# k-flouris/cmf

Hardware: AMD Instinct MI355X
Metric: log-density evals/sec (JtJ-cholesky path), MNIST D=784 d=64 bs=512 (higher is better)
Workload: dtype f32 (3x3 tangent convs as bf16x3 split MFMA, fp32 accumulate); 1 GPU; C3: MNIST-shaped (1,28,28) uint8-range + U[0,1) noise, non-square flow d=64, cholesky J^T J log-det + g_ij off-diagonal L1 + reconstruction, eval/no_grad; per_gpu_batch=512, global_batch=512, D=784, latent_dimension=64, parallelism=dp1

## Files before the change

### cmf_amd/csrc/conv_head.hip

```cpp
#include <stdint.h>

#include "common.h"

namespace {

constexpr int HID = 64, KJ = HID * 9, NT = 192, ACC = 16;
constexpr int SLICE = HID * 16;

__device__ __forceinline__ int out_pixel(int po, int W, int live) {
  if (!live) return po;
  const int wh = W >> 1, row = po / wh, k = po - row * wh;
  return row * W + 2 * k + ((row + live - 1) & 1);
}

template <int CP>
__global__ __launch_bounds__(NT, CP == 8 ? 2 : 3) void conv_head_kernel(cmf_conv_tangent_args a, int n_out, int tiles_per_sample, int ntiles) {
  constexpr int P = ACC / CP;
  __shared__ __attribute__((aligned(16))) float Es[P * KJ * CP];
  __shared__ __attribute__((aligned(16))) float Gs[HID * ACC];
  __shared__ unsigned long long um[P * 9];
  __shared__ unsigned long long alv[P];
  __shared__ int pixs[P];

  const int per = (ntiles + 7) >> 3;
  const int item = (int)(blockIdx.x & 7) * per + (int)(blockIdx.x >> 3);
  if (item >= ntiles) return;
  const int b = item / tiles_per_sample, p0 = (item - b * tiles_per_sample) * P;
  const int cnt = n_out - p0 < P ? n_out - p0 : P;
  const int tid = threadIdx.x, lane = tid & 63, wv = tid >> 6;
  const int H = a.H, W = a.W, cout = a.head_cout;

  if (tid < P * 9) {
    const int p = tid / 9, tap = tid - p * 9;
    unsigned long long m = 0;
    if (p < cnt) {
      const int pix = out_pixel(p0 + p, W, a.live);
      const int r = pix / W + tap / 3 - 1, c = pix % W + tap % 3 - 1;
      if (r >= 0 && r < H && c >= 0 && c < W)
        m = *reinterpret_cast<const unsigned long long*>(reinterpret_cast<const unsigned char*>(a.f) + (long long)b * a.f_np +
                                                         (long long)(r * W + c) * (HID / 8));
    }
    um[tid] = m;
  }
  for (int p = wv; p < P; p += NT / 64) {
    const int pix = p < cnt ? out_pixel(p0 + p, W, a.live) : 0;
    bool on = false;
    if (p < cnt) on = a.head_a[(long long)b * a.head_a_np + (long long)lane * a.head_a_c + (long long)pix * a.head_a_px] > 0.f;
    const unsigned long long bal = __ballot(on);
    if (lane == 0) {
      alv[p] = bal;
      pixs[p] = pix;
    }
#pragma unroll
    for (int o = 0; o < CP; ++o) Gs[(lane * P + p) * CP + o] = (on && o < cout) ? a.head_w[o * HID + lane] : 0.f;
  }
  __syncthreads();

  {
    static_assert(3 * NT == KJ, "three (ci, tap) pairs per thread");
    float acc[3][ACC];
#pragma unroll
    for (int r = 0; r < 3; ++r)
#pragma unroll
      for (int i = 0; i < ACC; ++i) acc[r][i] = 0.f;
#pragma unroll 2
    for (int c = 0; c < HID; ++c) {
      float w[3];
#pragma unroll
      for (int r = 0; r < 3; ++r) w[r] = a.w[c * KJ + tid + r * NT];
#pragma unroll
      for (int i = 0; i < ACC / 4; ++i) {
        const f32x4 g = *reinterpret_cast<const f32x4*>(&Gs[c * ACC + 4 * i]);
#pragma unroll
        for (int r = 0; r < 3; ++r)
#pragma unroll
          for (int k = 0; k < 4; ++k) acc[r][4 * i + k] = fmaf(g[k], w[r], acc[r][4 * i + k]);
      }
    }
#pragma unroll
    for (int r = 0; r < 3; ++r)
#pragma unroll
      for (int p = 0; p < P; ++p)
#pragma unroll
        for (int o = 0; o < CP; ++o) Es[(p * KJ + tid + r * NT) * CP + o] = acc[r][p * CP + o];
  }
  __syncthreads();

  const int nsl = a.nc >> 4, cl = lane >> 2;
  const f32x4 zero = {0.f, 0.f, 0.f, 0.f};
  for (int unit = wv; unit < nsl * P; unit += NT / 64) {
    const int sl = unit / P, p = unit - sl * P;
    if (p >= cnt) continue;
    const int pix = pixs[p];
    const float* hb = a.r + (long long)b * a.r_np + (long long)pix * a.r_px + sl * SLICE + lane * 4;
    const float* ub = a.x + (long long)b * a.x_np + sl * SLICE + lane * 4;
    f32x4 acc[CP];
#pragma unroll
    for (int o = 0; o < CP; ++o) acc[o] = zero;

    auto load4 = [&](f32x4* v, const float* src, unsigned long long m) {
#pragma unroll
      for (int ch = 0; ch < 4; ++ch) {
        v[ch] = zero;
        if ((m >> (ch * 16 + cl)) & 1) v[ch] = *reinterpret_cast<const f32x4*>(src + ch * 256);
      }
    };
    auto load_row = [&](f32x4* v, int ty) {
#pragma unroll
      for (int tx = 0; tx < 3; ++tx)
        load4(v + 4 * tx, ub + (long long)(pix + (ty - 1) * W + (tx - 1)) * a.x_px, um[p * 9 + ty * 3 + tx]);
    };
    auto fma4 = [&](const f32x4* v, const float* coef, int stride) {
#pragma unroll
      for (int ch = 0; ch < 4; ++ch) {
        const float* e4 = static_cast<const float*>(__builtin_assume_aligned(coef + ch * stride, CP < 4 ? 8 : 16));
#pragma unroll
        for (int o = 0; o < CP; ++o) {
          const float e = e4[o];
#pragma unroll
          for (int k = 0; k < 4; ++k) acc[o][k] = fmaf(e, v[ch][k], acc[o][k]);
        }
      }
    };
    auto fma_row = [&](const f32x4* v, int ty) {
#pragma unroll
      for (int tx = 0; tx < 3; ++tx) fma4(v + 4 * tx, &Es[(p * KJ + cl * 9 + ty * 3 + tx) * CP], 16 * 9 * CP);
    };
    {
      f32x4 vh[4], v[12];
      load4(vh, hb, alv[p]);
      load_row(v, 0);
      fma4(vh, &Gs[(cl * P + p) * CP], 16 * P * CP);
      fma_row(v, 0);
    }
#pragma unroll 1
    for (int ty = 1; ty < 3; ++ty) {
      f32x4 v[12];
      load_row(v, ty);
      fma_row(v, ty);
    }

    constexpr int N = 4 * CP;
    float val[N];
#pragma unroll
    for (int o = 0; o < CP; ++o)
#pragma unroll
      for (int k = 0; k < 4; ++k) val[4 * o + k] = acc[o][k];
#pragma unroll
    for (int s = 0; s < 4; ++s) {
      const int off = 32 >> s, n = N >> s;
      if (n >= 2) {
        const bool hi = lane & off;
#pragma unroll
        for (int i = 0; i < n / 2; ++i) {
          const float mine = hi ? val[n / 2 + i] : val[i], send = hi ? val[i] : val[n / 2 + i];
          val[i] = mine + __shfl_xor(send, off, 64);
        }
      } else {
        val[0] += __shfl_xor(val[0], off, 64);
      }
    }
    float* yb = a.head_y + (long long)b * a.head_y_np + (long long)(p0 + p) * a.head_y_px + sl * 16 + (lane & 3) * 4;
    constexpr int KEEP = N >= 16 ? N / 16 : 1;
#pragma unroll
    for (int i = 0; i < KEEP; ++i) {
      const int idx = ((cl * N) >> 4) + i, o = idx >> 2;
      if (o < cout && (N >= 16 || !(lane & 4))) yb[(long long)o * a.head_y_co + (idx & 3)] = val[i];
    }
  }
}

template <int CP>
int launch(const cmf_conv_tangent_args& a, hipStream_t s) {
  constexpr int P = ACC / CP;
  const int n_out = a.live ? a.H * a.W / 2 : a.H * a.W;
  const long long tiles = (n_out + P - 1) / P, ntiles = tiles * a.np;
  if (ntiles > 0x7ffffff0LL) return CMF_ERANGE;
  const int grid = 8 * (int)((ntiles + 7) / 8);
  hipLaunchKernelGGL(conv_head_kernel<CP>, dim3(grid), dim3(NT), 0, s, a, n_out, (int)tiles, (int)ntiles);
  CMF_LAUNCH_CHECK();
  return 0;
}

}

int cmf_conv_head(const cmf_conv_tangent_args& a, hipStream_t s) {
  if (!a.x || !a.w || !a.f || !a.r || !a.head_w || !a.head_a || !a.head_y) return CMF_EINVAL;
  if (a.fmode != CMF_F_RELU_BITS || a.taps != 9 || a.cin != HID || a.cout != HID) return CMF_EINVAL;
  if (a.head_cout < 1 || a.head_cout > 8 || a.np <= 0 || a.H <= 0 || a.W <= 0 || a.nc <= 0 || a.nc % 16) return CMF_EINVAL;
  if (a.bias || a.fo || a.ymask || a.mask_out || a.live < 0 || a.live > 2 || (a.live && a.W % 2)) return CMF_EINVAL;
  if (!((a.W % 14 == 0 && a.H % 2 == 0) || (a.W % 8 == 0 && a.H % 4 == 0))) return CMF_EINVAL;
  const long long HW = (long long)a.H * a.W;
  if (HW > (1 << 24)) return CMF_ERANGE;
  if (a.x_ci != 16 || a.x_sl != SLICE || a.r_co != 16 || a.r_sl != SLICE) return CMF_EINVAL;
  if ((a.x_np | a.x_px | a.r_np | a.r_px | a.head_y_np | a.head_y_co | a.head_y_px) % 4) return CMF_EINVAL;
  if (a.x_px < (long long)HID * a.nc || a.r_px < (long long)HID * a.nc || a.head_y_px < a.nc) return CMF_EINVAL;
  if ((uintptr_t)a.x % 16 || (uintptr_t)a.r % 16 || (uintptr_t)a.head_y % 16 || (uintptr_t)a.w % 4 || (uintptr_t)a.head_w % 4) return CMF_EINVAL;
  if ((uintptr_t)a.f % 8 || a.f_np % 8 || a.f_np < HW * (HID / 8)) return CMF_EINVAL;
  const int cp = a.head_cout <= 2 ? 2 : a.head_cout <= 4 ? 4 : 8;
  return cp == 2 ? launch<2>(a, s) : cp == 4 ? launch<4>(a, s) : launch<8>(a, s);
}
```

Baseline: 1489 evals/s.

## Deduplicate conv-head tap loads and pipeline them with a buffer-load ring

The conv head kernel now builds a per-tile table of unique input pixels shared across the P output pixels' 3x3 neighbourhoods, so overlapping taps are loaded once and applied to every output that uses them. Loads go through raw buffer_load instructions with out-of-range offsets standing in for masked lanes, issued into a three-deep register ring so global loads overlap FMA work. A fourth wave is added that prefetches while the other three compute the E coefficients, and the E layout in LDS is padded (stride 11) to hold the head weights as a tenth tap. This adds considerable complexity, inline asm with hand-set waitcnts, and higher register pressure under the same launch bounds.

Result: no change. 1492 evals/s (median of 6 runs) (+0.2%).

```diff
diff --git a/cmf_amd/csrc/conv_head.hip b/cmf_amd/csrc/conv_head.hip
--- a/cmf_amd/csrc/conv_head.hip
+++ b/cmf_amd/csrc/conv_head.hip
@@ -1,11 +1,19 @@
 #include <stdint.h>
 
+#include <type_traits>
+
 #include "common.h"
 
 namespace {
 
-constexpr int HID = 64, KJ = HID * 9, NT = 192, ACC = 16;
+constexpr int HID = 64, KJ = HID * 9, NT = 256, NW = NT / 64, NTB = 192, ACC = 16;
 constexpr int SLICE = HID * 16;
+constexpr int ES = 11;
+constexpr int RING = 3;
+constexpr int NENT = 128;
+constexpr int X_DROP = 0x7ffffff0;
+
+typedef int i32x4 __attribute__((ext_vector_type(4)));
 
 __device__ __forceinline__ int out_pixel(int po, int W, int live) {
   if (!live) return po;
@@ -13,51 +21,194 @@
   return row * W + 2 * k + ((row + live - 1) & 1);
 }
 
+__device__ __forceinline__ i32x4 block_rsrc(const float* p) {
+  const unsigned long long u = reinterpret_cast<unsigned long long>(p);
+  i32x4 d;
+  d[0] = __builtin_amdgcn_readfirstlane((int)(unsigned)u);
+  d[1] = __builtin_amdgcn_readfirstlane((int)((unsigned)(u >> 32) & 0xffffu));
+  d[2] = SLICE * 4;
+  d[3] = 0x00020000;
+  return d;
+}
+
 template <int CP>
 __global__ __launch_bounds__(NT, CP == 8 ? 2 : 3) void conv_head_kernel(cmf_conv_tangent_args a, int n_out, int tiles_per_sample, int ntiles) {
   constexpr int P = ACC / CP;
-  __shared__ __attribute__((aligned(16))) float Es[P * KJ * CP];
+  __shared__ __attribute__((aligned(16))) float Es[P * HID * ES * CP];
   __shared__ __attribute__((aligned(16))) float Gs[HID * ACC];
-  __shared__ unsigned long long um[P * 9];
-  __shared__ unsigned long long alv[P];
-  __shared__ int pixs[P];
+  __shared__ __attribute__((aligned(16))) unsigned ent[NENT][4];
+  __shared__ int keys[P * 9], fst[P * 9], nent_s;
 
   const int per = (ntiles + 7) >> 3;
   const int item = (int)(blockIdx.x & 7) * per + (int)(blockIdx.x >> 3);
   if (item >= ntiles) return;
   const int b = item / tiles_per_sample, p0 = (item - b * tiles_per_sample) * P;
   const int cnt = n_out - p0 < P ? n_out - p0 : P;
-  const int tid = threadIdx.x, lane = tid & 63, wv = tid >> 6;
+  const int tid = threadIdx.x, lane = tid & 63, wv = __builtin_amdgcn_readfirstlane(tid >> 6);
   const int H = a.H, W = a.W, cout = a.head_cout;
 
+  constexpr int NOKEY = 0x7fffffff;
+  const bool narrow = W + 2 <= 64;
+  int key = NOKEY, kq = 0;
+  unsigned long long km = 0;
   if (tid < P * 9) {
     const int p = tid / 9, tap = tid - p * 9;
-    unsigned long long m = 0;
     if (p < cnt) {
       const int pix = out_pixel(p0 + p, W, a.live);
       const int r = pix / W + tap / 3 - 1, c = pix % W + tap % 3 - 1;
-      if (r >= 0 && r < H && c >= 0 && c < W)
-        m = *reinterpret_cast<const unsigned long long*>(reinterpret_cast<const unsigned char*>(a.f) + (long long)b * a.f_np +
-                                                         (long long)(r * W + c) * (HID / 8));
-    }
-    um[tid] = m;
-  }
-  for (int p = wv; p < P; p += NT / 64) {
+      key = (r + 1) * (W + 2) + c + 1;
+      if (r >= 0 && r < H && c >= 0 && c < W) {
+        kq = r * W + c;
+        km = *reinterpret_cast<const unsigned long long*>(reinterpret_cast<const unsigned char*>(a.f) + (long long)b * a.f_np +
+                                                          (long long)kq * (HID / 8));
+      }
+      if (narrow) {
+        const int wh = a.live ? W >> 1 : W, row0 = p0 / wh;
+        int row = row0, k = p0 - row0 * wh;
+        unsigned long long rows[4] = {0, 0, 0, 0};
+        unsigned code = ~0u;
+#pragma unroll
+        for (int i = 0; i < P; ++i) {
+          if (i < cnt) {
+            const int col = a.live ? 2 * k + ((row + a.live - 1) & 1) : k, d = row - row0;
+            const unsigned long long w3 = 7ull << col;
+#pragma unroll
+            for (int x = 0; x < 4; ++x)
+              if (x >= d && x <= d + 2) rows[x] |= w3;
+            const int dr = r - row, dc = c - col;
+            if (dr >= -1 && dr <= 1 && dc >= -1 && dc <= 1) code = (code & ~(0xfu << (4 * i))) | ((unsigned)((dr + 1) * 3 + dc + 1) << (4 * i));
+            if (++k == wh) {
+              k = 0;
+              ++row;
+            }
+          }
+        }
+        const int rr = r - row0 + 1;
+        int rank = 0, n = 0;
+#pragma unroll
+        for (int x = 0; x < 4; ++x) {
+          n += __popcll(rows[x]);
+          rank += x < rr ? __popcll(rows[x]) : x == rr ? __popcll(rows[x] & ((1ull << (c + 1)) - 1)) : 0;
+        }
+        const int j = cnt + rank;
+        ent[j][0] = (unsigned)kq;
+        ent[j][1] = (unsigned)km;
+        ent[j][2] = (unsigned)(km >> 32);
+        ent[j][3] = code;
+        if (tid == 0) nent_s = cnt + n;
+      }
+    }
+    keys[tid] = key;
+  }
+  if (!narrow && tid >= cnt && tid < NENT) ent[tid][3] = ~0u;
+  for (int p = wv; p < P; p += NW) {
     const int pix = p < cnt ? out_pixel(p0 + p, W, a.live) : 0;
     bool on = false;
     if (p < cnt) on = a.head_a[(long long)b * a.head_a_np + (long long)lane * a.head_a_c + (long long)pix * a.head_a_px] > 0.f;
     const unsigned long long bal = __ballot(on);
-    if (lane == 0) {
-      alv[p] = bal;
-      pixs[p] = pix;
-    }
-#pragma unroll
-    for (int o = 0; o < CP; ++o) Gs[(lane * P + p) * CP + o] = (on && o < cout) ? a.head_w[o * HID + lane] : 0.f;
+    if (lane == 0 && p < cnt) {
+      ent[p][0] = (unsigned)pix | 0x80000000u;
+      ent[p][1] = (unsigned)bal;
+      ent[p][2] = (unsigned)(bal >> 32);
+      ent[p][3] = ~(0xfu << (4 * p)) | (9u << (4 * p));
+    }
+#pragma unroll
+    for (int o = 0; o < CP; ++o) {
+      const float g = (on && o < cout) ? a.head_w[o * HID + lane] : 0.f;
+      Gs[(lane * P + p) * CP + o] = g;
+      Es[((p * HID + lane) * ES + 9) * CP + o] = g;
+    }
   }
   __syncthreads();
-
-  {
-    static_assert(3 * NT == KJ, "three (ci, tap) pairs per thread");
+  if (!narrow) {
+    if (tid < P * 9) {
+      int first = key != NOKEY;
+      for (int t = 0; t < P * 9; ++t) first &= !(t < tid && keys[t] == key);
+      fst[tid] = first;
+    }
+    __syncthreads();
+    if (tid < P * 9) {
+      int rank = 0, n = 0;
+      for (int t = 0; t < P * 9; ++t) {
+        rank += fst[t] & (keys[t] < key);
+        n += fst[t];
+      }
+      if (tid == 0) nent_s = cnt + n;
+      if (key != NOKEY) {
+        const int p = tid / 9, tap = tid - p * 9, j = cnt + rank;
+        if (fst[tid]) {
+          ent[j][0] = (unsigned)kq;
+          ent[j][1] = (unsigned)km;
+          ent[j][2] = (unsigned)(km >> 32);
+        }
+        atomicAnd(&ent[j][3], ~(0xfu << (4 * p)) | ((unsigned)tap << (4 * p)));
+      }
+    }
+    __syncthreads();
+  }
+
+  const int nsl = a.nc >> 4;
+  const int nent = __builtin_amdgcn_readfirstlane(nent_s);
+  const int lsub = nsl >= 3 ? 0 : nsl == 2 ? 1 : (P < NW ? 1 : 2);
+  const int psub = P >> lsub, nunits = nsl << lsub;
+  const i32x4 e0 = *reinterpret_cast<const i32x4*>(ent[lane]), e1 = *reinterpret_cast<const i32x4*>(ent[lane + 64]);
+  auto field = [&](int j, int k) {
+    if constexpr (P * 10 <= 64) {
+      return (unsigned)__builtin_amdgcn_readlane(e0[k], j);
+    } else {
+      const int lo = __builtin_amdgcn_readlane(e0[k], j & 63), hi = __builtin_amdgcn_readlane(e1[k], j & 63);
+      return (unsigned)(j < 64 ? lo : hi);
+    }
+  };
+  auto others = [&](int u) { return ~(unsigned)(((1ull << (4 * psub)) - 1) << (4 * psub * (u & ((1 << lsub) - 1)))); };
+  const f32x4 zero = {0.f, 0.f, 0.f, 0.f};
+  int lcl = lane >> 2;
+  asm volatile("" : "+v"(lcl));
+  const int loff = lane * 16;
+  const unsigned bit0 = 1u << lcl, bit1 = 0x10000u << lcl;
+  const long long xpx = a.x_px, rpx = a.r_px;
+  f32x4 ring[RING][4];
+  int iu = wv, ij = 0;
+  const float *ixb = a.x, *irb = a.r;
+  unsigned iot = 0;
+  auto issue_unit = [&]() {
+    const int u = iu < nunits ? iu : 0;
+    ixb = a.x + (long long)b * a.x_np + (u >> lsub) * SLICE;
+    irb = a.r + (long long)b * a.r_np + (u >> lsub) * SLICE;
+    iot = others(u);
+  };
+  issue_unit();
+  auto issue = [&](f32x4 (&v)[4]) {
+    const bool valid = iu < nunits;
+    const int j = valid ? ij : 0;
+    const unsigned e = field(j, 0);
+    const bool need = valid && (lsub == 0 || (field(j, 3) | iot) != ~0u);
+    const unsigned mlo = need ? field(j, 1) : 0u, mhi = need ? field(j, 2) : 0u;
+    const long long pixel = (long long)(e & 0x7fffffffu);
+    const float* src = (e >> 31) ? irb + pixel * rpx : ixb + pixel * xpx;
+    const i32x4 rs = block_rsrc(src);
+    const int o0 = mlo & bit0 ? loff : X_DROP, o1 = mlo & bit1 ? loff : X_DROP;
+    const int o2 = mhi & bit0 ? loff : X_DROP, o3 = mhi & bit1 ? loff : X_DROP;
+    asm volatile(
+        "s_nop 4\n\t"
+        "buffer_load_dwordx4 %0, %4, %8, 0 offen\n\t"
+        "buffer_load_dwordx4 %1, %5, %8, 0 offen offset:1024\n\t"
+        "buffer_load_dwordx4 %2, %6, %8, 0 offen offset:2048\n\t"
+        "buffer_load_dwordx4 %3, %7, %8, 0 offen offset:3072"
+        : "=&v"(v[0]), "=&v"(v[1]), "=&v"(v[2]), "=&v"(v[3])
+        : "v"(o0), "v"(o1), "v"(o2), "v"(o3), "s"(rs)
+        : "memory");
+    if (valid && ++ij == nent) {
+      ij = 0;
+      iu += NW;
+      issue_unit();
+    }
+  };
+#pragma unroll
+  for (int s = 0; s < RING; ++s) issue(ring[s]);
+
+  if (tid < NTB) {
+    static_assert(3 * NTB == KJ, "three (ci, tap) pairs per thread");
     float acc[3][ACC];
 #pragma unroll
     for (int r = 0; r < 3; ++r)
@@ -67,7 +218,7 @@
     for (int c = 0; c < HID; ++c) {
       float w[3];
 #pragma unroll
-      for (int r = 0; r < 3; ++r) w[r] = a.w[c * KJ + tid + r * NT];
+      for (int r = 0; r < 3; ++r) w[r] = a.w[c * KJ + tid + r * NTB];
 #pragma unroll
       for (int i = 0; i < ACC / 4; ++i) {
         const f32x4 g = *reinterpret_cast<const f32x4*>(&Gs[c * ACC + 4 * i]);
@@ -78,96 +229,106 @@
       }
     }
 #pragma unroll
-    for (int r = 0; r < 3; ++r)
+    for (int r = 0; r < 3; ++r) {
+      const int pair = tid + r * NTB, ci = pair / 9, tap = pair - ci * 9;
 #pragma unroll
       for (int p = 0; p < P; ++p)
 #pragma unroll
-        for (int o = 0; o < CP; ++o) Es[(p * KJ + tid + r * NT) * CP + o] = acc[r][p * CP + o];
+        for (int o = 0; o < CP; ++o) Es[((p * HID + ci) * ES + tap) * CP + o] = acc[r][p * CP + o];
+    }
   }
   __syncthreads();
 
-  const int nsl = a.nc >> 4, cl = lane >> 2;
-  const f32x4 zero = {0.f, 0.f, 0.f, 0.f};
-  for (int unit = wv; unit < nsl * P; unit += NT / 64) {
-    const int sl = unit / P, p = unit - sl * P;
-    if (p >= cnt) continue;
-    const int pix = pixs[p];
-    const float* hb = a.r + (long long)b * a.r_np + (long long)pix * a.r_px + sl * SLICE + lane * 4;
-    const float* ub = a.x + (long long)b * a.x_np + sl * SLICE + lane * 4;
-    f32x4 acc[CP];
-#pragma unroll
-    for (int o = 0; o < CP; ++o) acc[o] = zero;
-
-    auto load4 = [&](f32x4* v, const float* src, unsigned long long m) {
-#pragma unroll
-      for (int ch = 0; ch < 4; ++ch) {
-        v[ch] = zero;
-        if ((m >> (ch * 16 + cl)) & 1) v[ch] = *reinterpret_cast<const f32x4*>(src + ch * 256);
+  f32x4 acc[P][CP];
+#pragma unroll
+  for (int p = 0; p < P; ++p)
+#pragma unroll
+    for (int o = 0; o < CP; ++o) acc[p][o] = zero;
+  auto finish = [&](int u) {
+    const int sl = u >> lsub, pa = (u & ((1 << lsub) - 1)) * psub, pb = pa + psub < cnt ? pa + psub : cnt;
+    int ln = lane;
+    asm volatile("" : "+v"(ln));
+    const int cf = ln >> 2;
+#pragma unroll
+    for (int p = 0; p < P; ++p) {
+      if (p >= pa && p < pb) {
+        constexpr int N = 4 * CP;
+        float val[N];
+#pragma unroll
+        for (int o = 0; o < CP; ++o)
+#pragma unroll
+          for (int k = 0; k < 4; ++k) val[4 * o + k] = acc[p][o][k];
+#pragma unroll
+        for (int s = 0; s < 4; ++s) {
+          const int off = 32 >> s, n = N >> s;
+          if (n >= 2) {
+            const bool hi = ln & off;
+#pragma unroll
+            for (int i = 0; i < n / 2; ++i) {
+              const float mine = hi ? val[n / 2 + i] : val[i], send = hi ? val[i] : val[n / 2 + i];
+              val[i] = mine + __shfl_xor(send, off, 64);
+            }
+          } else {
+            val[0] += __shfl_xor(val[0], off, 64);
+          }
+        }
+        float* yb = a.head_y + (long long)b * a.head_y_np + (long long)(p0 + p) * a.head_y_px + sl * 16 + (ln & 3) * 4;
+        constexpr int KEEP = N >= 16 ? N / 16 : 1;
+#pragma unroll
+        for (int i = 0; i < KEEP; ++i) {
+          const int idx = ((cf * N) >> 4) + i, o = idx >> 2;
+          if (o < cout && (N >= 16 || !(ln & 4))) yb[(long long)o * a.head_y_co + (idx & 3)] = val[i];
+        }
+      }
+#pragma unroll
+      for (int o = 0; o < CP; ++o) acc[p][o] = zero;
+    }
+  };
+  int cu = wv, cj = 0;
+  unsigned cot = others(cu);
+  auto consume = [&](f32x4 (&v)[4]) {
+    asm volatile("s_waitcnt vmcnt(%4)" : "+v"(v[0]), "+v"(v[1]), "+v"(v[2]), "+v"(v[3]) : "n"(4 * (RING - 1)));
+    const unsigned code = field(cj, 3) | cot;
+    const int lb = lcl * (ES * CP);
+    auto feed = [&](auto pc) {
+      constexpr int p = decltype(pc)::value;
+      const int nib = (code >> (4 * p)) & 15;
+      if (nib != 15) {
+#pragma unroll
+        for (int ch = 0; ch < 4; ++ch) {
+          const float* e4 = static_cast<const float*>(
+              __builtin_assume_aligned(&Es[(p * HID + ch * 16) * ES * CP + lb + nib * CP], CP < 4 ? 8 : 16));
+#pragma unroll
+          for (int o = 0; o < CP; ++o) {
+            const float w = e4[o];
+#pragma unroll
+            for (int k = 0; k < 4; ++k) acc[p][o][k] = fmaf(w, v[ch][k], acc[p][o][k]);
+          }
+        }
       }
     };
-    auto load_row = [&](f32x4* v, int ty) {
-#pragma unroll
-      for (int tx = 0; tx < 3; ++tx)
-        load4(v + 4 * tx, ub + (long long)(pix + (ty - 1) * W + (tx - 1)) * a.x_px, um[p * 9 + ty * 3 + tx]);
-    };
-    auto fma4 = [&](const f32x4* v, const float* coef, int stride) {
-#pragma unroll
-      for (int ch = 0; ch < 4; ++ch) {
-        const float* e4 = static_cast<const float*>(__builtin_assume_aligned(coef + ch * stride, CP < 4 ? 8 : 16));
-#pragma unroll
-        for (int o = 0; o < CP; ++o) {
-          const float e = e4[o];
-#pragma unroll
-          for (int k = 0; k < 4; ++k) acc[o][k] = fmaf(e, v[ch][k], acc[o][k]);
-        }
-      }
-    };
-    auto fma_row = [&](const f32x4* v, int ty) {
-#pragma unroll
-      for (int tx = 0; tx < 3; ++tx) fma4(v + 4 * tx, &Es[(p * KJ + cl * 9 + ty * 3 + tx) * CP], 16 * 9 * CP);
-    };
-    {
-      f32x4 vh[4], v[12];
-      load4(vh, hb, alv[p]);
-      load_row(v, 0);
-      fma4(vh, &Gs[(cl * P + p) * CP], 16 * P * CP);
-      fma_row(v, 0);
-    }
-#pragma unroll 1
-    for (int ty = 1; ty < 3; ++ty) {
-      f32x4 v[12];
-      load_row(v, ty);
-      fma_row(v, ty);
-    }
-
-    constexpr int N = 4 * CP;
-    float val[N];
-#pragma unroll
-    for (int o = 0; o < CP; ++o)
-#pragma unroll
-      for (int k = 0; k < 4; ++k) val[4 * o + k] = acc[o][k];
-#pragma unroll
-    for (int s = 0; s < 4; ++s) {
-      const int off = 32 >> s, n = N >> s;
-      if (n >= 2) {
-        const bool hi = lane & off;
-#pragma unroll
-        for (int i = 0; i < n / 2; ++i) {
-          const float mine = hi ? val[n / 2 + i] : val[i], send = hi ? val[i] : val[n / 2 + i];
-          val[i] = mine + __shfl_xor(send, off, 64);
-        }
-      } else {
-        val[0] += __shfl_xor(val[0], off, 64);
-      }
-    }
-    float* yb = a.head_y + (long long)b * a.head_y_np + (long long)(p0 + p) * a.head_y_px + sl * 16 + (lane & 3) * 4;
-    constexpr int KEEP = N >= 16 ? N / 16 : 1;
-#pragma unroll
-    for (int i = 0; i < KEEP; ++i) {
-      const int idx = ((cl * N) >> 4) + i, o = idx >> 2;
-      if (o < cout && (N >= 16 || !(lane & 4))) yb[(long long)o * a.head_y_co + (idx & 3)] = val[i];
-    }
-  }
+    if ((code & 0xffu) != 0xffu) feed(std::integral_constant<int, 0>{}), feed(std::integral_constant<int, 1>{});
+    if constexpr (P > 2)
+      if ((code & 0xff00u) != 0xff00u) feed(std::integral_constant<int, 2>{}), feed(std::integral_constant<int, 3>{});
+    if constexpr (P > 4) {
+      if ((code & 0xff0000u) != 0xff0000u) feed(std::integral_constant<int, 4>{}), feed(std::integral_constant<int, 5>{});
+      if ((code & 0xff000000u) != 0xff000000u) feed(std::integral_constant<int, 6>{}), feed(std::integral_constant<int, 7>{});
+    }
+    issue(v);
+    if (++cj == nent) {
+      finish(cu);
+      cj = 0;
+      cu += NW;
+      cot = others(cu);
+    }
+  };
+  const int total = cu < nunits ? (nunits - cu + NW - 1) / NW * nent : 0;
+  for (int step = 0; step < total; step += RING) {
+#pragma unroll
+    for (int s = 0; s < RING; ++s)
+      if (step + s < total) consume(ring[s]);
+  }
+  asm volatile("s_waitcnt vmcnt(0)" ::: "memory");
 }
 
 template <int CP>
```
